# NVIDIA/nvidia-resiliency-ext

Measured on AMD Instinct MI355X. Metric: generate_report_latency_us, lower is better.
Workload: dtype f32; 1 GPU; 8 ranks x 64 sections x 10000 samples per report, ring capacity 10000, relative+individual scores, gather_on_rank0; logical_ranks_per_gpu=8, rows_per_gpu=512, exchange=none (single process)

## Files before the change

### include/nvrx_straggler.h

```cpp
#ifndef NVRX_STRAGGLER_H
#define NVRX_STRAGGLER_H

#include <stddef.h>
#include <stdint.h>

#ifdef __cplusplus
extern "C" {
#endif

#define NVRX_ABI_VERSION 2

#define NVRX_OK 0
#define NVRX_ERR_INVALID (-22)
#define NVRX_ERR_NOMEM (-12)
#define NVRX_ERR_HIP (-5)
#define NVRX_ERR_STATE (-1)
#define NVRX_ERR_RANGE (-34)
#define NVRX_ERR_TIMEOUT (-62)

#define NVRX_STATS_STRIDE 8
#define NVRX_STAT_MIN 0
#define NVRX_STAT_MAX 1
#define NVRX_STAT_MED 2
#define NVRX_STAT_AVG 3
// ... 175 lines not shown
    float *d_stats_dst;
    uint32_t *d_done_counter;
    void *allgather_fn;
    void *comm;
    int32_t send_count;
    uint32_t seq;
    const uint32_t *h_seq_word;
    double timeout_s;
    void *order_after_stream;
    int32_t order_after_enabled;
    int32_t resident;
    int32_t prev_settled;
    int32_t guard_rings;
} nvrx_report_desc;
int nvrx_report(nvrx_ctx *ctx, nvrx_report_desc *desc, void *stream);
int nvrx_report_attribute(nvrx_ctx *ctx, const nvrx_report_desc *desc, int first_rank, int n_ranks, int top_n, void *d_out);
int nvrx_tail_local(nvrx_ctx *ctx, const nvrx_report_desc *desc, uint32_t q_ppm, float *d_tail_send, int K, int S,
                    int rows_active, void *stream);
int nvrx_onset_enable(nvrx_ctx *ctx, int on);
int nvrx_onset_local(nvrx_ctx *ctx, const nvrx_report_desc *desc, uint32_t min_seg_ppm, float min_strength,
                     float *d_onset_send, int K, int S, int rows_active, void *stream);
int nvrx_period_local(nvrx_ctx *ctx, const nvrx_report_desc *desc, int max_period, float min_strength,
                      float *d_period_send, int K, int S, int rows_active, void *stream);
int nvrx_episode_local(nvrx_ctx *ctx, const nvrx_report_desc *desc, uint32_t min_len_ppm, float min_strength,
                       float *d_episode_send, int K, int S, int rows_active, void *stream);
int nvrx_report_robust(nvrx_ctx *ctx, const nvrx_report_desc *desc, int first_rank, int n_ranks, int min_ranks,
                       float floor_rel, void *d_out);
int nvrx_report_peer(nvrx_ctx *ctx, const nvrx_report_desc *desc, const int32_t *d_groups, int G, int first_rank, int n_ranks,
                     int min_ranks, void *d_out);
int nvrx_report_pace(nvrx_ctx *ctx, const nvrx_report_desc *desc, int first_rank, int n_ranks, int min_ranks, void *d_out);
// ... 15 lines not shown
#define NVRX_WINDOW_MISS 1
#define NVRX_WINDOW_NAMES 2
typedef struct nvrx_window_desc {
    int (*kt_sync)(double timeout_s);
    int (*kt_hold)(int on);
    uint64_t (*kt_counter)(int what);
    double kt_patience_s;
    uint64_t kt_rows_known;
    uint64_t kt_keys_without_row;
    int32_t rows_used;
    int32_t asynchronous;
    int32_t harvest_regions;
    int32_t out_names_ok;
} nvrx_window_desc;
int nvrx_window_report(nvrx_ctx *ctx, nvrx_report_desc *desc, void *stream, nvrx_window_desc *window);
int nvrx_window_clocks(double *out2);
int nvrx_report_clocks(double *out8);
int nvrx_report_desc_size(void);
typedef struct nvrx_peer nvrx_peer;
int nvrx_peer_create(int device, int world, int rank, int max_floats_per_rank, nvrx_peer **out);
int nvrx_peer_ipc_handle(nvrx_peer *peer, void *handle64 );
int nvrx_peer_connect(nvrx_peer *peer, int peer_rank, const void *handle64);
int nvrx_peer_device_id(const nvrx_peer *peer, char *out, int len);
int nvrx_peer_check_access(const nvrx_peer *peer, int peer_rank, const char *peer_pci_bus_id);
int nvrx_peer_ready(nvrx_peer *peer, double timeout_s);
int nvrx_peer_allgather(const void *send, void *recv, size_t count, int dtype, void *comm, void *stream);
void *nvrx_peer_allgather_address(void);
int nvrx_peer_error(const nvrx_peer *peer, uint32_t *epoch_out);
int nvrx_peer_destroy(nvrx_peer *peer);

// ... 19 lines not shown
```

### nvidia-resiliency-ext_amd/csrc/nvrx_straggler.hip

```cpp
#include <hip/hip_runtime.h>
#include <hip/hip_ext.h>

#include <algorithm>
#include <atomic>
#include <chrono>
#include <thread>
#include <cmath>
#include <cstdarg>
#include <cstdio>
#include <cstdlib>
#include <cstring>
#include <deque>
#include <mutex>
#include <string>
#include <unordered_map>
#include <utility>
#include <vector>

#include "nvrx_straggler.h"

namespace {

thread_local std::string g_err;

// ... 1691 lines not shown
    hipEvent_t order_ev = nullptr;
    hipStream_t score_stream = nullptr;
    unsigned long long *d_rowg = nullptr;
    uint32_t *h_gather_err = nullptr, *d_gather_err = nullptr;
    uint32_t gran_epoch = 0;
    int wall_khz = 100000;
    int resident_mode = 1;
    int poll_naps = 4;
    int rehome_mode = 1;
    bool side_work = true;
    uint64_t reports_rehomed = 0;
    int last_rehome_verdict = 0;
    uint64_t side_gen = 1, async_gen = 0;
    bool async_on_ctx = false;
    double last_report_us = 0.0;
    double async_rehome_gap_us = 5000.0;
    hipEvent_t report_ev = nullptr;
    uint64_t report_epoch = 0;
    hipStream_t guard_stream = nullptr;
    bool guard_recorded = true;
    bool stamps_used = false;
    uint64_t guard_done_epoch = 0;
    struct StreamEpoch {
        hipStream_t stream;
        uint64_t epoch;
    };
    std::vector<StreamEpoch> stream_epochs;

    const nvrx_report_desc *attr_desc = nullptr;
    hipStream_t attr_stream = nullptr;
// ... 1171 lines not shown
    a->rank = p->rank;
    a->count = (int)count;
    a->stride = p->stride;
    p->epoch = (p->epoch % 0x7FFFFFFFu) + 1u;
    a->epoch = p->epoch;
    a->timeout_ticks = (unsigned long long)(p->timeout_s * 1e3 * (double)p->wall_khz);
    return NVRX_OK;
}

int nvrx_report_clocks(double *out8) {
    if (!out8) return fail(NVRX_ERR_INVALID, "null argument");
    memcpy(out8, g_report_clk, sizeof(g_report_clk));
    return NVRX_OK;
}

int nvrx_report(nvrx_ctx *ctx, nvrx_report_desc *d, void *stream) {
    report_clk(0);
    if (!ctx || !d) return fail(NVRX_ERR_INVALID, "null argument");
    if (!d->d_stats || !d->d_send || !d->d_scores || !d->d_meta) return fail(NVRX_ERR_INVALID, "null buffer in the report descriptor");
    const bool exchanging = d->allgather_fn != nullptr;
    if (exchanging && (!d->d_table || d->d_table == d->d_send || d->send_count <= 0))
        return fail(NVRX_ERR_INVALID, "an exchange needs a separate table buffer and a positive send_count");
    const bool is_async = d->h_seq_word == nullptr;
    bool async_gap_ok = false;
    {
        std::lock_guard<std::mutex> lk(ctx->mu);
        const double now_us = g_report_clk[0];
        async_gap_ok = ctx->async_rehome_gap_us > 0.0 && ctx->last_report_us > 0.0 && now_us - ctx->last_report_us >= ctx->async_rehome_gap_us;
        ctx->last_report_us = now_us;
        ctx->last_rehome_verdict = 0;
        if (d->prev_settled) {
            ctx->guard_done_epoch = ctx->report_epoch;
            if (ctx->async_on_ctx && ctx->async_gen == ctx->side_gen) ctx->side_work = false;
            ctx->async_on_ctx = false;
        }
    }
    bool rehomed = false;
    if (ctx->rehome_mode && ((!is_async && !d->guard_rings) || (is_async && d->guard_rings && async_gap_ok))) {
        std::lock_guard<std::mutex> lk(ctx->mu);
        hipStream_t only = nullptr;
        int distinct = 0;
// ... 88 lines not shown
        ga.timeout_ticks = (unsigned long long)((d->timeout_s > 0.0 ? d->timeout_s : 1e9) * 1e3 * (double)ctx->wall_khz);
        ga.poll_naps = ctx->poll_naps;
        PeerArgs pa{};
        if (peer_route) {
            rc2 = peer_fill_args(static_cast<nvrx_peer *>(d->comm), d->d_send, d->d_table, (size_t)d->send_count, &pa);
            if (rc2) return rc2;
        }
        d->seq = (d->seq % 0x7FFFFFFFu) + 1u;
        rc2 = score_launch(exchanging ? d->d_table : d->d_send, d->R, d->K, d->S, d->do_indiv, d->do_rel, d->thresholds,
                           d->d_scores, d->d_flags, d->d_meta, d->d_done_counter, d->seq, nullptr, nullptr, 0,
                           ctx->score_stream, peer_route ? &pa : nullptr, &ga);
        if (rc2) return rc2;
        ctx->attr_desc = d, ctx->attr_stream = ctx->score_stream;
        report_clk(4);
        report_clk(5);
        rc2 = nvrx_poll_u32(d->h_seq_word, d->seq, d->timeout_s > 0.0 ? d->timeout_s : 1e30);
        report_clk(6);
        if (rc2) return rc2;
        if (*static_cast<volatile uint32_t *>(ctx->h_gather_err) == ctx->gran_epoch)
            return fail(NVRX_ERR_TIMEOUT, "the score kernel gave up waiting for the statistics kernel's rows (epoch %u)", ctx->gran_epoch);
        if (as_stream(stream) == ctx->default_stream) {
            std::lock_guard<std::mutex> lk(ctx->mu);
            ctx->side_work = false;
            ctx->async_on_ctx = false;
        }
        return NVRX_OK;
    }
    int rc = report_local_impl(ctx, d->d_stats, d->d_send, d->K, d->S, d->names_ok, d->rows_active, stream, nullptr, 0);
    if (rc) return rc;
    if (d->guard_rings) {
        std::lock_guard<std::mutex> lk(ctx->mu);
        ctx->guard_stream = as_stream(stream);
        if (rehomed || !ctx->stamps_used) {
            ctx->guard_recorded = false;
        } else {
            HIP_TRY(hipEventRecord(ctx->report_ev, as_stream(stream)));
            ctx->guard_recorded = true;
        }
        ctx->report_epoch++;
    }
// ... 9 lines not shown
        const int nrc = reinterpret_cast<AllGatherFn>(d->allgather_fn)(d->d_send, d->d_table, (size_t)d->send_count, 7,
                                                                       d->comm, stream);
        if (nrc != 0) {
            return fail(NVRX_ERR_HIP, "all-gather of the exchange rows failed (ncclResult %d)", nrc);
        }
    }
    report_clk(4);
    d->seq = (d->seq % 0x7FFFFFFFu) + 1u;
    rc = score_launch(exchanging ? d->d_table : d->d_send, d->R, d->K, d->S, d->do_indiv, d->do_rel, d->thresholds,
                      d->d_scores, d->d_flags, d->d_meta, d->d_done_counter, d->seq, d->d_stats, d->d_stats_dst,
                      d->stats_rows, stream, prologue ? &pa : nullptr);
    if (rc) return rc;
    ctx->attr_desc = d, ctx->attr_stream = as_stream(stream);
    report_clk(5);
    if (d->h_seq_word) {
        rc = nvrx_poll_u32(d->h_seq_word, d->seq, d->timeout_s > 0.0 ? d->timeout_s : 1e30);
        report_clk(6);
        if (rc == NVRX_OK && !rehomed && as_stream(stream) == ctx->default_stream) {
            std::lock_guard<std::mutex> lk(ctx->mu);
            ctx->side_work = false;
            ctx->async_on_ctx = false;
        }
        return rc;
    }
    if (!rehomed) {
        std::lock_guard<std::mutex> lk(ctx->mu);
        ctx->async_on_ctx = true;
        ctx->async_gen = ctx->side_gen;
    }
    return NVRX_OK;
}

static thread_local double g_window_clk[2] = {0.0, 0.0};

int nvrx_window_clocks(double *out2) {
    if (!out2) return fail(NVRX_ERR_INVALID, "out2 is null");
    out2[0] = g_window_clk[0], out2[1] = g_window_clk[1];
    return NVRX_OK;
}

int nvrx_window_report(nvrx_ctx *ctx, nvrx_report_desc *desc, void *stream, nvrx_window_desc *w) {
    if (!ctx || !desc || !w) return fail(NVRX_ERR_INVALID, "null argument");
    g_window_clk[0] = g_window_clk[1] = std::chrono::duration<double, std::micro>(std::chrono::steady_clock::now().time_since_epoch()).count();
    const bool per_kernel = w->kt_sync != nullptr;
    if (per_kernel && (!w->kt_hold || !w->kt_counter)) return fail(NVRX_ERR_INVALID, "a kernel tracer needs sync, hold and counter");
    const bool enqueue_only = w->asynchronous != 0;
    bool held = false;
    auto leave = [&](int rc) {
        if (held) w->kt_hold(0);
        return rc;
    };
    w->out_names_ok = 1;
    if (per_kernel) {
        if (enqueue_only) {
            w->kt_hold(1);
            held = true;
// ... 11 lines not shown
    {
        const int n = w->rows_used;
        bool bad = false, changed = false;
        {
            std::lock_guard<std::mutex> lk(ctx->mu);
            bad = n < 0 || n > ctx->rows;
            if (!bad) {
                changed = ctx->occupied_rows != n;
                for (int r = 0; r < n && !changed; r++) changed = ctx->occupied_seen[(size_t)r] != (uint8_t)(ctx->total[(size_t)r] != 0);
            }
        }
        if (bad) return leave(fail(NVRX_ERR_INVALID, "rows_used %d outside [0,%d]", n, ctx->rows));
        if (changed) return leave(NVRX_WINDOW_MISS);
    }
    g_window_clk[1] = std::chrono::duration<double, std::micro>(std::chrono::steady_clock::now().time_since_epoch()).count();
    const int rc = nvrx_report(ctx, desc, stream);
    if (rc < 0) return leave(rc);
    if (!enqueue_only && desc->h_seq_word) {
        const uint32_t names = *const_cast<const volatile uint32_t *>(desc->h_seq_word - 4);
        if (names != 1u) {
            w->out_names_ok = 0;
            return leave(NVRX_WINDOW_NAMES);
        }
    }
    const int rrc = nvrx_ring_reset(ctx);
    return leave(rrc < 0 ? rrc : NVRX_OK);
}

int nvrx_peer_create(int device, int world, int rank, int max_floats_per_rank, nvrx_peer **out) {
    if (!out) return fail(NVRX_ERR_INVALID, "out is null");
// ... 275 lines not shown
```

### nvidia-resiliency-ext_amd/nvrx_straggler/_native.py

```python
from __future__ import annotations

import ctypes
import os
import threading
from ctypes import POINTER, c_char_p, c_double, c_float, c_int, c_int32, c_size_t, c_uint32, c_uint64, c_void_p

_LIB_NAME = "libnvrx_straggler_hip.so"
_LIB_PATH = os.path.join(os.environ.get("NVRX_DEBUG_LIB_DIR") or os.path.join(os.path.dirname(os.path.abspath(__file__)), "lib"), _LIB_NAME)

NVRX_ABI_VERSION = 2
STATS_STRIDE = 8
STAT_MIN, STAT_MAX, STAT_MED, STAT_AVG, STAT_STD, STAT_NUM, STAT_WEIGHT = range(7)
KIND_SECTION, KIND_KERNEL = 0, 1
MAX_RING_CAP = 65536
META_WORDS = 8
ERR_TIMEOUT = -62
ERR_RANGE = -34
ERR_INVALID = -22
ERR_STATE = -1
ATTR_MAX_TOP = 16
TAIL_Q_PPM_MIN, TAIL_Q_PPM_MAX = 500000, 999999
ROUTE_SINGLE, ROUTE_ROWS, ROUTE_ROWS_PRE, ROUTE_TILE16, ROUTE_TILE8 = 1, 2, 3, 4, 5
ROBUST_MAX_RANKS = 65536
PEER_MAX_GROUPS = 4096
# ... 89 lines not shown
    ("nvrx_row_configure", c_int, [c_void_p, c_int, c_int, c_int]),
    ("nvrx_ring_push", c_int, [c_void_p, c_int, c_float]),
    ("nvrx_ring_push_many", c_int, [c_void_p, c_int, c_void_p, c_int]),
    ("nvrx_ring_push_pairs", c_int, [c_void_p, c_void_p, c_void_p, c_int]),
    ("nvrx_ring_push_staged", c_int, [c_void_p, c_void_p, c_void_p, c_int]),
    ("nvrx_sink_push", c_int, [c_void_p, c_void_p, c_void_p, c_int]),
    ("nvrx_sink_row_alloc", c_int, [c_void_p, c_int]),
    ("nvrx_ring_push_device", c_int, [c_void_p, c_int, c_void_p, c_int, c_void_p]),
    ("nvrx_ring_push_device_rows", c_int, [c_void_p, c_int, c_int, c_void_p, c_int, c_int, c_void_p]),
    ("nvrx_ring_set_count", c_int, [c_void_p, c_int, c_int]),
    ("nvrx_ring_set_count_all", c_int, [c_void_p, c_int]),
    ("nvrx_ring_count", c_int, [c_void_p, c_int]),
    ("nvrx_ring_counts", c_int, [c_void_p, c_void_p, c_int]),
    ("nvrx_ring_occupancy_changed", c_int, [c_void_p, c_int]),
    ("nvrx_window_report", c_int, [c_void_p, c_void_p, c_void_p, c_void_p]),
    ("nvrx_window_clocks", c_int, [POINTER(c_double)]),
    ("nvrx_ring_reset", c_int, [c_void_p]),
    ("nvrx_history_reset", c_int, [c_void_p, c_void_p]),
    ("nvrx_ring_flush", c_int, [c_void_p, c_void_p]),
    ("nvrx_ring_read", c_int, [c_void_p, c_int, c_void_p, c_int, c_void_p]),
    ("nvrx_event_begin", c_int, [c_void_p, c_int, c_void_p]),
    ("nvrx_event_end", c_int, [c_void_p, c_int, c_void_p]),
    ("nvrx_event_harvest", c_int, [c_void_p, c_int]),
    ("nvrx_stamp_begin", c_int, [c_void_p, c_int, c_void_p]),
    ("nvrx_stamp_end", c_int, [c_void_p, c_int, c_int, c_float, c_void_p]),
    ("nvrx_report_local", c_int, [c_void_p, c_void_p, c_void_p, c_int, c_int, c_int, c_int, c_void_p]),
    ("nvrx_report", c_int, [c_void_p, POINTER(ReportDesc), c_void_p]),
    ("nvrx_report_attribute", c_int, [c_void_p, POINTER(ReportDesc), c_int, c_int, c_int, c_void_p]),
    ("nvrx_tail_local", c_int, [c_void_p, POINTER(ReportDesc), c_uint32, c_void_p, c_int, c_int, c_int, c_void_p]),
    ("nvrx_onset_enable", c_int, [c_void_p, c_int]),
    ("nvrx_onset_local", c_int, [c_void_p, POINTER(ReportDesc), c_uint32, c_float, c_void_p, c_int, c_int, c_int, c_void_p]),
    ("nvrx_period_local", c_int, [c_void_p, POINTER(ReportDesc), c_int, c_float, c_void_p, c_int, c_int, c_int, c_void_p]),
    ("nvrx_episode_local", c_int, [c_void_p, POINTER(ReportDesc), c_uint32, c_float, c_void_p, c_int, c_int, c_int, c_void_p]),
    ("nvrx_report_robust", c_int, [c_void_p, POINTER(ReportDesc), c_int, c_int, c_int, c_float, c_void_p]),
    ("nvrx_report_peer", c_int, [c_void_p, POINTER(ReportDesc), c_void_p, c_int, c_int, c_int, c_int, c_void_p]),
    ("nvrx_report_pace", c_int, [c_void_p, POINTER(ReportDesc), c_int, c_int, c_int, c_void_p]),
    ("nvrx_report_pace_group", c_int, [c_void_p, POINTER(ReportDesc), c_void_p, c_int, c_int, c_int, c_int, c_int, c_int,
                                       c_void_p]),
    ("nvrx_report_node", c_int, [c_void_p, POINTER(ReportDesc), c_void_p, c_int, c_int, c_int, c_int, c_int, c_int, c_void_p]),
    ("nvrx_report_history", c_int, [c_void_p, POINTER(ReportDesc), c_int, c_int, c_void_p, c_int, c_int, c_uint64,
                                    POINTER(c_double), c_void_p]),
    ("nvrx_report_trend", c_int, [c_void_p, c_void_p, c_int, c_int, c_int, c_int, c_uint64, c_void_p]),
# ... 225 lines not shown
```

### nvidia-resiliency-ext_amd/nvrx_straggler/backend.py

```python
from __future__ import annotations

import ctypes
import os
import threading
import weakref
from typing import Any, Dict, List, Optional, Sequence

import numpy as np
import torch

from . import _native
from .row_families import EPISODE, FAMILIES, ONSET, PERIOD, TAIL, RowFamily
from .table_families import NODE, PACE, PACE_GROUP, PEER, ROBUST, SLOTS, TableFamily

DEFAULT_THRESHOLDS = (0.75, 0.75, 0.75, 0.75)



def report_timeout_s() -> float:
    t = _timeout_cache[0]
    if t is None:
        t = refresh_report_timeout()
    return t

# ... 1399 lines not shown
        d.rows_active, d.stats_rows = rows_active, min(stats_rows, ws.stats_rows)
        d.do_indiv, d.do_rel = int(do_indiv), int(do_rel)
        d.names_ok = int(names_ok)
        for i in range(4):
            d.thresholds[i] = float(thresholds[i])
        if direct is not None:
            d.allgather_fn, d.comm = direct.fn_address, direct.comm_address
        else:
            d.allgather_fn, d.comm = None, None
        d.timeout_s = report_timeout_s()
        d.h_seq_word = blk.h_seq if wait else None
        d.guard_rings = 0 if wait else 1
        d.resident = 1 if (wait and resident) else 0
        blk.desc_key = key

    def report_fused(self, ws: Workspace, rows_active: int, stats_rows: int, do_indiv: bool, do_rel: bool,
                     thresholds: Sequence[float], direct=None, names_ok: bool = True, wait: bool = True,
                     order_after: Optional[int] = None, resident: bool = True, prev_settled: bool = False) -> int:
        blk = ws.flip()
        d = blk.desc
        key = (rows_active, stats_rows, do_indiv, do_rel, thresholds, direct, names_ok, wait, resident)
        if blk.desc_key != key:
            self.configure_desc(ws, blk, key)
        d.prev_settled = 1 if (prev_settled and not wait) else 0
        if order_after is not None:
            d.order_after_stream, d.order_after_enabled = order_after, 1
        elif d.order_after_enabled:
            d.order_after_enabled = 0
        if not ws.send_initialised:
            self.backend.send_init(ws)
            self.backend.synchronize()
        d.seq = ws.seq
        rc = self.lib.nvrx_report(self.ctx, blk.desc_ref, self.backend._stream_handle)
        ws.seq = d.seq
        if rc < 0:
            if rc == _native.ERR_TIMEOUT:
                self.backend.retire_workspace(ws)
            _native.check(rc)
        return ws.seq

    def report_attribute(self, ws: Workspace, top_n: int, first_rank: int = 0, n_ranks: Optional[int] = None) -> Attribution:
        n_ranks = ws.R - first_rank if n_ranks is None else n_ranks
        ws.attr_settle()
        buf, _ = ws.attr_buffers(n_ranks, top_n, False)
        rc = self.lib.nvrx_report_attribute(self.ctx, ws.block.desc_ref, first_rank, n_ranks, top_n, buf.data_ptr())
        if rc < 0:
            _native.check(rc)
        out = ws._attr_last = Attribution(self.backend, buf, first_rank, n_ranks, top_n)
        return out

    def _table_report(self, fam: TableFamily, ws: Workspace, groups: Optional[PeerGroups], first_rank: int,
                      n_ranks: Optional[int], params: tuple) -> TableScores:
        return self.backend._table_step(fam, ws, getattr(self.lib, fam.c_report), (self.ctx, ws.block.desc_ref), (), groups,
                                        first_rank, n_ranks, params)
# ... 127 lines not shown
```

### nvidia-resiliency-ext_amd/nvrx_straggler/reporting.py

```python
from __future__ import annotations

import collections
import dataclasses
import itertools
import logging
import math
import os
import threading
import time
from typing import Any, Dict, List, Mapping, Optional, Sequence

import numpy as np

from . import backend as _backend_mod
from . import dist_utils, row_families
from .name_mapper import NameMapper, name_digest
from .statistics import NUM_COLUMN, STAT_KEYS, Statistic

_SummaryType = Mapping[Statistic, float]
_LOG = logging.getLogger(__name__)



def _load_pyread():
# ... 1597 lines not shown
        self.rank = dist_utils.get_rank(self.group)
        self.node_name = node_name
        self.thresholds = tuple(float(t) for t in thresholds)

        self.min_local_kernel_times: Dict[str, float] = collections.defaultdict(lambda: float("inf"))
        self.min_local_section_times: Dict[str, float] = collections.defaultdict(lambda: float("inf"))

        self.name_mapper = NameMapper(pg=pg)
        self._private_mapper = NameMapper(pg=pg)
        self.rank_to_node: Dict[int, str] = collections.defaultdict(lambda: "<unk>")
        self._rank_to_node_folded = False
        self._direct = None
        self._direct_tried = False
        self.asynchronous = bool(asynchronous)
        self.exchange_info: Dict[str, Any] = {}
        self._ring_plan = None
        self._ring_gid_state = None
        self._inflight: Optional[_PendingBlock] = None
        self._prev_async_settled = True
        self._resync_pending = False
        self._had_ring_report = False
        self._unreported_rows: list = []
        n = int(kernel_attribution)
        if not 0 <= n <= 16:
            raise ValueError(f"kernel_attribution must be 0 (off) or 1..16 kernels per GPU score, got {kernel_attribution!r}")
        self.kernel_attribution = n
        if n:
            be = _backend_mod._backend
            if be is not None and not hasattr(be, "attribute"):
                raise RuntimeError(f"kernel_attribution={n}: the active backend ({getattr(be, 'name', type(be).__name__)}) "
# ... 658 lines not shown
            raise RuntimeError("peer_groups: these rings run the one-call report but have no report_peer")
        if fused and self.pace_scores and not hasattr(rings, "report_pace_group" if self.pace_peer_groups else "report_pace"):
            if self.pace_peer_groups:
                raise RuntimeError("pace_peer_groups: these rings run the one-call report but have no report_pace_group")
            raise RuntimeError("pace_scores: these rings run the one-call report but have no report_pace")
        if fused and self.node_scores and not hasattr(rings, "report_node"):
            raise RuntimeError("node_scores: these rings run the one-call report but have no report_node")
        if fused and self._peer_history is not None and not hasattr(rings, "report_peer_history"):
            raise RuntimeError("peer_history: these rings run the one-call report but have no report_peer_history")
        if fused and self.peer_trends and not hasattr(rings, "report_peer_trend"):
            raise RuntimeError("peer_trends: these rings run the one-call report but have no report_peer_trend")
        if fused and self._history is not None and not hasattr(rings, "report_history"):
            raise RuntimeError("score_history: these rings run the one-call report but have no report_history")
        if fused and self.score_trends and not hasattr(rings, "report_trend"):
            raise RuntimeError("score_trends: these rings run the one-call report but have no report_trend")
        if fused:
            wait = not self.asynchronous
            seq = rings.report_fused(ws, plan.rows_used, plan.stats_needed, self.is_computing_indiv_scores,
                                     self.is_computing_rel_scores, self.thresholds, self._direct if multi else None,
                                     names_ok=names_ok, wait=wait, order_after=order_after if multi else None,
                                     resident=not (multi and getattr(self._direct, "shared_device", False)
                                                   and os.environ.get("NVRX_DEBUG_RESIDENT_SHARED_OK", "0") in ("", "0")),
                                     prev_settled=self._prev_async_settled)
            if not wait:
                self._prev_async_settled = False
                pend = self._inflight = _PendingBlock(be, ws, seq)
                if self.gather_on_rank0 and self.rank != 0:
                    return None
                report = Report._from_device(
                    _ScoreSource(plan.view, pend),
                    self._shared_rank_to_node(),
                    (time.perf_counter_ns() - t0) * 1e-6, self.gather_on_rank0, self.rank)
                if attr_n:
                    self._attach_plan_attribution(report, plan, rings, True)
                if self.robust_scores:
                    self._attach_plan_robust(report, plan, rings, True)
                if self.work_groups:
                    self._attach_plan_work(report, plan, rings, True)
                if self.peer_groups is not None:
                    self._attach_plan_peer(report, plan, rings, True)
                if self.pace_scores:
                    self._attach_plan_pace(report, plan, rings, True)
                if self.node_scores:
                    self._attach_plan_node(report, plan, rings, True)
                if self._history is not None:
                    self._attach_plan_history(report, plan, rings, True)
                return report
        else:
            rings.report_local(ws, True, rows_active=plan.rows_used)
            table = self._exchange(be, ws) if multi else ws.send
            be.score(ws, table, self.is_computing_indiv_scores, self.is_computing_rel_scores, self.thresholds,
                     wait=True, stats_rows=plan.stats_needed)
        if fused:
            mark = getattr(ws, "mark_live", None)
            if mark is not None:
                mark(ws.seq)
        if multi:
            self._check_exchange()
        if ws.meta[0] != 1:
            return False
        if self.gather_on_rank0 and self.rank != 0:
            return None
        if fused:
            pending = _LiveBlock(be, ws, ws.seq, plan.stats_needed)
            ws.attach(pending)
        else:
            pending = ws.host_block()
        report = Report._from_device(
            _ScoreSource(plan.view, pending),
            self._shared_rank_to_node(),
            (time.perf_counter_ns() - t0) * 1e-6, self.gather_on_rank0, self.rank)
        if attr_n:
            self._attach_plan_attribution(report, plan, rings, fused)
        if self.robust_scores:
            self._attach_plan_robust(report, plan, rings, fused)
        if self.work_groups:
            self._attach_plan_work(report, plan, rings, fused)
        if self.peer_groups is not None:
            self._attach_plan_peer(report, plan, rings, fused)
        if self.pace_scores:
            self._attach_plan_pace(report, plan, rings, fused)
        if self.node_scores:
            self._attach_plan_node(report, plan, rings, fused)
        if self._history is not None:
            self._attach_plan_history(report, plan, rings, fused)
        return report
# ... 368 lines not shown
```

### nvidia-resiliency-ext_amd/nvrx_straggler/straggler.py

```python
from __future__ import annotations

import ctypes
import dataclasses
import functools
import inspect
import logging
import os
import socket
import sys
import time
from collections.abc import Callable
from contextlib import contextmanager
from typing import Any, Dict, Iterable, List, Optional, Sequence, Union

from . import _native, row_families
from . import backend as _backend_mod
from . import dist_utils as _dist_utils
from . import ktrace as _ktrace
from .cupti import CuptiManager
from .interval_tracker import ReportIntervalTracker
from .reporting import Report, ReportGenerator, _LiveBlock, _PendingBlock, _ScoreSource
from .statistics import Statistic

GPU_KEY_PREFIX = "hipevent::"
# ... 57 lines not shown
        self.row = rings.row_for(_native.KIND_SECTION, name)
        self.gpu_row: Optional[int] = None
        self.cpu_elapsed_times = _ElapsedRing(rings, self.row)


_MISS = object()
_TRACED_DISPATCH_US = 1.0


class _Lane:

    trace = None

    __slots__ = ("rings", "reporter", "manager", "ext", "plan", "ws", "be", "view", "versions", "wr", "group", "wr_cache",
                 "rows_used", "desc_key", "window", "window_ref", "call", "ctx", "stream", "multi", "enqueue_only",
                 "returns_none", "stats_needed", "gather_on_rank0", "rank", "token", "asynchronous")

    @classmethod
    def build(cls, det) -> Optional["_Lane"]:
        rings, reporter, manager = det._rings, det.reporter, det._cupti_manager
        plan = reporter._ring_plan
        call = getattr(getattr(rings, "lib", None), "nvrx_window_report", None)
        if plan is None or not plan.fused or call is None or manager is None or not manager.is_initialized:
            return None
        multi = reporter.world_size > 1 and reporter._exchanged()
        if (multi and reporter._direct is None) or det._pending_region_switch is not None:
            return None
        if reporter.asynchronous and not reporter.enqueue_only():
            return None
        if reporter.kernel_attribution:
            return None
# ... 37 lines not shown
        if manager.per_kernel:
            if not getattr(ext, "_counting", False):
                return None
            cast, klib = ctypes.cast, ext._lib
            w.kt_sync = cast(klib.nvrx_ktrace_sync, ctypes.c_void_p).value
            w.kt_hold = cast(klib.nvrx_ktrace_hold, ctypes.c_void_p).value
            w.kt_counter = cast(klib.nvrx_ktrace_counter, ctypes.c_void_p).value
            w.kt_patience_s = float(ext.sync_patience_s)
            w.kt_rows_known, w.kt_keys_without_row = int(ext._rows_known), int(ext.keys_without_row)
        else:
            w.harvest_regions = 1
        w.rows_used = self.rows_used
        w.asynchronous = 1 if self.enqueue_only else 0
        self.window_ref = ctypes.byref(w)
        self.call, self.ctx, self.stream = call, rings.ctx, self.be._stream_handle
        return self

    def run(self, det):
        t0 = time.perf_counter_ns()
        tr = _Lane.trace
        reporter, ws, rings = self.reporter, self.ws, self.rings
        if (reporter._ring_plan is not self.plan or rings._rows_used != self.rows_used or reporter._resync_pending
                or reporter.asynchronous is not self.asynchronous
                or (reporter.name_mapper.version, reporter._private_mapper.version) != self.versions
                or _dist_utils.world_and_rank(self.group, self.wr_cache) != self.wr):
            return _MISS
        if self.enqueue_only:
            pend = reporter._inflight
            if pend is not None:
                blk = pend.blk
# ... 16 lines not shown
        if nxt.desc_key != self.desc_key:
            rings.configure_desc(ws, nxt, self.desc_key)
        if nxt._live is not None:
            nxt.settle()
        ws._cur, ws.block = 1 - cur, nxt
        d = nxt.desc
        if self.enqueue_only:
            d.prev_settled = 1 if reporter._prev_async_settled else 0
        if self.multi:
            d.order_after_stream, d.order_after_enabled = self.be.current_stream_handle(), 1
        elif d.order_after_enabled:
            d.order_after_enabled = 0
        d.seq = ws.seq
        if tr is not None:
            tr.append(("settle_flip_desc", time.perf_counter_ns() - t0))
        rc = self.call(self.ctx, nxt.desc_ref, self.stream, self.window_ref)
        if tr is not None:
            tr.append(("c_call", time.perf_counter_ns() - t0))
        seq = ws.seq = d.seq
        if rc == _native.WINDOW_MISS:
            ws._cur, ws.block = cur, ws.blocks[cur]
            return _MISS
        if rc < 0:
            reporter._drop_plan()
            if rc == _native.ERR_TIMEOUT:
                self.be.retire_workspace(ws)
            _native.check(rc)
        if self.enqueue_only:
            reporter._prev_async_settled = False
            pend = reporter._inflight = _PendingBlock(self.be, ws, seq)
# ... 5 lines not shown
        if self.multi:
            reporter._check_exchange()
        if rc == _native.WINDOW_NAMES:
            reporter._sync_names_first()
            return det._report_and_reset(rings, reporter)
        if self.returns_none:
            return None
        live = _LiveBlock(self.be, ws, seq, self.stats_needed)
        nxt.attach(live)
        if tr is not None:
            tr.append(("live_block", time.perf_counter_ns() - t0))
        rep = Report._from_device(_ScoreSource(self.view, live), reporter._shared_rank_to_node(),
                                  (time.perf_counter_ns() - t0) * 1e-6, self.gather_on_rank0, self.rank)
        if tr is not None:
            tr.append(("report_object", time.perf_counter_ns() - t0))
        return rep


def _peer_groups_from_env(value: str, name: str = "NVRX_PEER_GROUPS"):
    value = value.strip()
    if not value:
        return None
    if ":" in value or value == "auto":
        return value
    try:
        return [int(x) for x in value.split(",")]
    except ValueError:
        raise ValueError(f"{name} must be 'block:N', 'mod:N' or a comma-separated list of integers, "
                         f"got {value!r}") from None

# ... 629 lines not shown
```

Measured before the change: 26.24 us.

## Split synchronous report into enqueue and wait to overlap host object construction

Splits nvrx_report and nvrx_window_report into enqueue and wait/finish halves, keeping per-context pending state. The Python lane and reporter now enqueue the GPU report, build the Report and live-block objects while the kernels run, and only then poll the completion word. This hides the host-side Python object construction behind GPU execution. The cost is extra state-machine complexity, a new error path when a wait is missed, and the need for try/finally cleanup.

```diff
diff --git a/include/nvrx_straggler.h b/include/nvrx_straggler.h
--- a/include/nvrx_straggler.h
+++ b/include/nvrx_straggler.h
@@ -213,6 +213,8 @@
     int32_t guard_rings;
 } nvrx_report_desc;
 int nvrx_report(nvrx_ctx *ctx, nvrx_report_desc *desc, void *stream);
+int nvrx_report_enqueue(nvrx_ctx *ctx, nvrx_report_desc *desc, void *stream);
+int nvrx_report_wait(nvrx_ctx *ctx, nvrx_report_desc *desc);
 int nvrx_report_attribute(nvrx_ctx *ctx, const nvrx_report_desc *desc, int first_rank, int n_ranks, int top_n, void *d_out);
 int nvrx_tail_local(nvrx_ctx *ctx, const nvrx_report_desc *desc, uint32_t q_ppm, float *d_tail_send, int K, int S,
                     int rows_active, void *stream);
@@ -258,6 +260,8 @@
     int32_t out_names_ok;
 } nvrx_window_desc;
 int nvrx_window_report(nvrx_ctx *ctx, nvrx_report_desc *desc, void *stream, nvrx_window_desc *window);
+int nvrx_window_enqueue(nvrx_ctx *ctx, nvrx_report_desc *desc, void *stream, nvrx_window_desc *window);
+int nvrx_window_finish(nvrx_ctx *ctx, nvrx_report_desc *desc, nvrx_window_desc *window);
 int nvrx_window_clocks(double *out2);
 int nvrx_report_clocks(double *out8);
 int nvrx_report_desc_size(void);
diff --git a/nvidia-resiliency-ext_amd/csrc/nvrx_straggler.hip b/nvidia-resiliency-ext_amd/csrc/nvrx_straggler.hip
--- a/nvidia-resiliency-ext_amd/csrc/nvrx_straggler.hip
+++ b/nvidia-resiliency-ext_amd/csrc/nvrx_straggler.hip
@@ -1729,6 +1729,10 @@
     uint64_t side_gen = 1, async_gen = 0;
     bool async_on_ctx = false;
     double last_report_us = 0.0;
+    bool pend_on = false;
+    bool pend_resident = false, pend_rehomed = false;
+    hipStream_t pend_stream = nullptr;
+    uint32_t pend_seq = 0;
     double async_rehome_gap_us = 5000.0;
     hipEvent_t report_ev = nullptr;
     uint64_t report_epoch = 0;
@@ -2930,7 +2934,54 @@
     return NVRX_OK;
 }
 
+static void report_set_pending(nvrx_ctx *ctx, const nvrx_report_desc *d, bool resident, bool rehomed, hipStream_t st) {
+    std::lock_guard<std::mutex> lk(ctx->mu);
+    ctx->pend_on = true;
+    ctx->pend_resident = resident, ctx->pend_rehomed = rehomed;
+    ctx->pend_stream = st;
+    ctx->pend_seq = d->seq;
+}
+
 int nvrx_report(nvrx_ctx *ctx, nvrx_report_desc *d, void *stream) {
+    const int rc = nvrx_report_enqueue(ctx, d, stream);
+    if (rc || !d->h_seq_word) return rc;
+    return nvrx_report_wait(ctx, d);
+}
+
+int nvrx_report_wait(nvrx_ctx *ctx, nvrx_report_desc *d) {
+    if (!ctx || !d) return fail(NVRX_ERR_INVALID, "null argument");
+    if (!d->h_seq_word) return NVRX_OK;
+    bool resident = false, rehomed = false;
+    hipStream_t st = nullptr;
+    uint32_t seq = 0;
+    {
+        std::lock_guard<std::mutex> lk(ctx->mu);
+        if (!ctx->pend_on) return fail(NVRX_ERR_STATE, "nvrx_report_wait: no enqueued report is waiting on this context");
+        resident = ctx->pend_resident, rehomed = ctx->pend_rehomed, st = ctx->pend_stream, seq = ctx->pend_seq;
+        ctx->pend_on = false;
+    }
+    int rc = nvrx_poll_u32(d->h_seq_word, seq, d->timeout_s > 0.0 ? d->timeout_s : 1e30);
+    report_clk(6);
+    if (resident) {
+        if (rc) return rc;
+        if (*static_cast<volatile uint32_t *>(ctx->h_gather_err) == ctx->gran_epoch)
+            return fail(NVRX_ERR_TIMEOUT, "the score kernel gave up waiting for the statistics kernel's rows (epoch %u)", ctx->gran_epoch);
+        if (st == ctx->default_stream) {
+            std::lock_guard<std::mutex> lk(ctx->mu);
+            ctx->side_work = false;
+            ctx->async_on_ctx = false;
+        }
+        return NVRX_OK;
+    }
+    if (rc == NVRX_OK && !rehomed && st == ctx->default_stream) {
+        std::lock_guard<std::mutex> lk(ctx->mu);
+        ctx->side_work = false;
+        ctx->async_on_ctx = false;
+    }
+    return rc;
+}
+
+int nvrx_report_enqueue(nvrx_ctx *ctx, nvrx_report_desc *d, void *stream) {
     report_clk(0);
     if (!ctx || !d) return fail(NVRX_ERR_INVALID, "null argument");
     if (!d->d_stats || !d->d_send || !d->d_scores || !d->d_meta) return fail(NVRX_ERR_INVALID, "null buffer in the report descriptor");
@@ -2941,6 +2992,8 @@
     bool async_gap_ok = false;
     {
         std::lock_guard<std::mutex> lk(ctx->mu);
+        if (ctx->pend_on)
+            return fail(NVRX_ERR_STATE, "report %u was enqueued on this context and has not been waited for (nvrx_report_wait)", ctx->pend_seq);
         const double now_us = g_report_clk[0];
         async_gap_ok = ctx->async_rehome_gap_us > 0.0 && ctx->last_report_us > 0.0 && now_us - ctx->last_report_us >= ctx->async_rehome_gap_us;
         ctx->last_report_us = now_us;
@@ -3059,16 +3112,7 @@
         ctx->attr_desc = d, ctx->attr_stream = ctx->score_stream;
         report_clk(4);
         report_clk(5);
-        rc2 = nvrx_poll_u32(d->h_seq_word, d->seq, d->timeout_s > 0.0 ? d->timeout_s : 1e30);
-        report_clk(6);
-        if (rc2) return rc2;
-        if (*static_cast<volatile uint32_t *>(ctx->h_gather_err) == ctx->gran_epoch)
-            return fail(NVRX_ERR_TIMEOUT, "the score kernel gave up waiting for the statistics kernel's rows (epoch %u)", ctx->gran_epoch);
-        if (as_stream(stream) == ctx->default_stream) {
-            std::lock_guard<std::mutex> lk(ctx->mu);
-            ctx->side_work = false;
-            ctx->async_on_ctx = false;
-        }
+        report_set_pending(ctx, d, true, rehomed, as_stream(stream));
         return NVRX_OK;
     }
     int rc = report_local_impl(ctx, d->d_stats, d->d_send, d->K, d->S, d->names_ok, d->rows_active, stream, nullptr, 0);
@@ -3108,14 +3152,8 @@
     ctx->attr_desc = d, ctx->attr_stream = as_stream(stream);
     report_clk(5);
     if (d->h_seq_word) {
-        rc = nvrx_poll_u32(d->h_seq_word, d->seq, d->timeout_s > 0.0 ? d->timeout_s : 1e30);
-        report_clk(6);
-        if (rc == NVRX_OK && !rehomed && as_stream(stream) == ctx->default_stream) {
-            std::lock_guard<std::mutex> lk(ctx->mu);
-            ctx->side_work = false;
-            ctx->async_on_ctx = false;
-        }
-        return rc;
+        report_set_pending(ctx, d, false, rehomed, as_stream(stream));
+        return NVRX_OK;
     }
     if (!rehomed) {
         std::lock_guard<std::mutex> lk(ctx->mu);
@@ -3133,7 +3171,35 @@
     return NVRX_OK;
 }
 
+static int window_report_impl(nvrx_ctx *ctx, nvrx_report_desc *desc, void *stream, nvrx_window_desc *w, bool finish);
+
 int nvrx_window_report(nvrx_ctx *ctx, nvrx_report_desc *desc, void *stream, nvrx_window_desc *w) {
+    return window_report_impl(ctx, desc, stream, w, true);
+}
+
+int nvrx_window_enqueue(nvrx_ctx *ctx, nvrx_report_desc *desc, void *stream, nvrx_window_desc *w) {
+    if (!ctx || !desc || !w) return fail(NVRX_ERR_INVALID, "null argument");
+    if (w->asynchronous != 0 || !desc->h_seq_word)
+        return fail(NVRX_ERR_INVALID, "nvrx_window_enqueue is for synchronous windows (asynchronous ones: nvrx_window_report)");
+    return window_report_impl(ctx, desc, stream, w, false);
+}
+
+int nvrx_window_finish(nvrx_ctx *ctx, nvrx_report_desc *desc, nvrx_window_desc *w) {
+    if (!ctx || !desc || !w) return fail(NVRX_ERR_INVALID, "null argument");
+    if (w->asynchronous != 0 || !desc->h_seq_word)
+        return fail(NVRX_ERR_INVALID, "nvrx_window_finish is for synchronous windows (asynchronous ones: nvrx_window_report)");
+    const int rc = nvrx_report_wait(ctx, desc);
+    if (rc < 0) return rc;
+    const uint32_t names = *const_cast<const volatile uint32_t *>(desc->h_seq_word - 4);
+    if (names != 1u) {
+        w->out_names_ok = 0;
+        return NVRX_WINDOW_NAMES;
+    }
+    const int rrc = nvrx_ring_reset(ctx);
+    return rrc < 0 ? rrc : NVRX_OK;
+}
+
+static int window_report_impl(nvrx_ctx *ctx, nvrx_report_desc *desc, void *stream, nvrx_window_desc *w, bool finish) {
     if (!ctx || !desc || !w) return fail(NVRX_ERR_INVALID, "null argument");
     g_window_clk[0] = g_window_clk[1] = std::chrono::duration<double, std::micro>(std::chrono::steady_clock::now().time_since_epoch()).count();
     const bool per_kernel = w->kt_sync != nullptr;
@@ -3175,6 +3241,7 @@
         if (changed) return leave(NVRX_WINDOW_MISS);
     }
     g_window_clk[1] = std::chrono::duration<double, std::micro>(std::chrono::steady_clock::now().time_since_epoch()).count();
+    if (!finish) return leave(nvrx_report_enqueue(ctx, desc, stream));
     const int rc = nvrx_report(ctx, desc, stream);
     if (rc < 0) return leave(rc);
     if (!enqueue_only && desc->h_seq_word) {
diff --git a/nvidia-resiliency-ext_amd/csrc/split_report_args_check.cpp b/nvidia-resiliency-ext_amd/csrc/split_report_args_check.cpp
--- /dev/null
+++ b/nvidia-resiliency-ext_amd/csrc/split_report_args_check.cpp
@@ -0,0 +1,60 @@
+#include "args_check.h"
+
+static int sync_stub(double) { return 0; }
+
+int main() {
+    nvrx_ctx *ctx = reinterpret_cast<nvrx_ctx *>(uintptr_t{4096});
+    float *buf = reinterpret_cast<float *>(uintptr_t{8192});
+    uint32_t word[8] = {0, 0, 0, 0, 0, 0, 0, 0};
+    nvrx_report_desc d;
+    memset(&d, 0, sizeof(d));
+    nvrx_window_desc w;
+    memset(&w, 0, sizeof(w));
+
+    expect("enqueue null ctx", nvrx_report_enqueue(nullptr, &d, nullptr), NVRX_ERR_INVALID, "null");
+    expect("enqueue null desc", nvrx_report_enqueue(ctx, nullptr, nullptr), NVRX_ERR_INVALID, "null");
+    expect("enqueue null buffers", nvrx_report_enqueue(ctx, &d, nullptr), NVRX_ERR_INVALID, "null buffer");
+    expect("report null buffers", nvrx_report(ctx, &d, nullptr), NVRX_ERR_INVALID, "null buffer");
+    d.d_stats = d.d_send = d.d_scores = buf;
+    expect("enqueue null meta", nvrx_report_enqueue(ctx, &d, nullptr), NVRX_ERR_INVALID, "null buffer");
+    d.d_meta = reinterpret_cast<uint32_t *>(buf);
+    d.allgather_fn = reinterpret_cast<void *>(&sync_stub);
+    expect("enqueue exchange without a table", nvrx_report_enqueue(ctx, &d, nullptr), NVRX_ERR_INVALID, "table");
+    d.d_table = d.d_send;
+    d.send_count = 8;
+    expect("enqueue exchange into the send rows", nvrx_report_enqueue(ctx, &d, nullptr), NVRX_ERR_INVALID, "table");
+    d.d_table = buf + 1024;
+    d.send_count = 0;
+    expect("enqueue exchange of nothing", nvrx_report_enqueue(ctx, &d, nullptr), NVRX_ERR_INVALID, "send_count");
+    d.allgather_fn = nullptr;
+
+    expect("wait null ctx", nvrx_report_wait(nullptr, &d), NVRX_ERR_INVALID, "null");
+    expect("wait null desc", nvrx_report_wait(ctx, nullptr), NVRX_ERR_INVALID, "null");
+    d.h_seq_word = nullptr;
+    expect("wait on an asynchronous descriptor", nvrx_report_wait(ctx, &d), NVRX_OK, nullptr);
+
+    d.h_seq_word = &word[4];
+    expect("window enqueue null ctx", nvrx_window_enqueue(nullptr, &d, nullptr, &w), NVRX_ERR_INVALID, "null");
+    expect("window enqueue null desc", nvrx_window_enqueue(ctx, nullptr, nullptr, &w), NVRX_ERR_INVALID, "null");
+    expect("window enqueue null window", nvrx_window_enqueue(ctx, &d, nullptr, nullptr), NVRX_ERR_INVALID, "null");
+    w.asynchronous = 1;
+    expect("window enqueue asynchronous", nvrx_window_enqueue(ctx, &d, nullptr, &w), NVRX_ERR_INVALID, "synchronous");
+    w.asynchronous = 0;
+    d.h_seq_word = nullptr;
+    expect("window enqueue without a completion word", nvrx_window_enqueue(ctx, &d, nullptr, &w), NVRX_ERR_INVALID, "synchronous");
+    d.h_seq_word = &word[4];
+    w.kt_sync = &sync_stub;
+    expect("window enqueue half a tracer", nvrx_window_enqueue(ctx, &d, nullptr, &w), NVRX_ERR_INVALID, "tracer");
+    w.kt_sync = nullptr;
+
+    expect("window finish null ctx", nvrx_window_finish(nullptr, &d, &w), NVRX_ERR_INVALID, "null");
+    expect("window finish null desc", nvrx_window_finish(ctx, nullptr, &w), NVRX_ERR_INVALID, "null");
+    expect("window finish null window", nvrx_window_finish(ctx, &d, nullptr), NVRX_ERR_INVALID, "null");
+    w.asynchronous = 1;
+    expect("window finish asynchronous", nvrx_window_finish(ctx, &d, &w), NVRX_ERR_INVALID, "synchronous");
+    w.asynchronous = 0;
+    d.h_seq_word = nullptr;
+    expect("window finish without a completion word", nvrx_window_finish(ctx, &d, &w), NVRX_ERR_INVALID, "synchronous");
+    printf("split_report_args_check: %d failure(s)\n", failures);
+    return failures ? 1 : 0;
+}
diff --git a/nvidia-resiliency-ext_amd/nvrx_straggler/_native.py b/nvidia-resiliency-ext_amd/nvrx_straggler/_native.py
--- a/nvidia-resiliency-ext_amd/nvrx_straggler/_native.py
+++ b/nvidia-resiliency-ext_amd/nvrx_straggler/_native.py
@@ -127,6 +127,8 @@
     ("nvrx_ring_counts", c_int, [c_void_p, c_void_p, c_int]),
     ("nvrx_ring_occupancy_changed", c_int, [c_void_p, c_int]),
     ("nvrx_window_report", c_int, [c_void_p, c_void_p, c_void_p, c_void_p]),
+    ("nvrx_window_enqueue", c_int, [c_void_p, c_void_p, c_void_p, c_void_p]),
+    ("nvrx_window_finish", c_int, [c_void_p, c_void_p, c_void_p]),
     ("nvrx_window_clocks", c_int, [POINTER(c_double)]),
     ("nvrx_ring_reset", c_int, [c_void_p]),
     ("nvrx_history_reset", c_int, [c_void_p, c_void_p]),
@@ -139,6 +141,8 @@
     ("nvrx_stamp_end", c_int, [c_void_p, c_int, c_int, c_float, c_void_p]),
     ("nvrx_report_local", c_int, [c_void_p, c_void_p, c_void_p, c_int, c_int, c_int, c_int, c_void_p]),
     ("nvrx_report", c_int, [c_void_p, POINTER(ReportDesc), c_void_p]),
+    ("nvrx_report_enqueue", c_int, [c_void_p, POINTER(ReportDesc), c_void_p]),
+    ("nvrx_report_wait", c_int, [c_void_p, POINTER(ReportDesc)]),
     ("nvrx_report_attribute", c_int, [c_void_p, POINTER(ReportDesc), c_int, c_int, c_int, c_void_p]),
     ("nvrx_tail_local", c_int, [c_void_p, POINTER(ReportDesc), c_uint32, c_void_p, c_int, c_int, c_int, c_void_p]),
     ("nvrx_onset_enable", c_int, [c_void_p, c_int]),
diff --git a/nvidia-resiliency-ext_amd/nvrx_straggler/backend.py b/nvidia-resiliency-ext_amd/nvrx_straggler/backend.py
--- a/nvidia-resiliency-ext_amd/nvrx_straggler/backend.py
+++ b/nvidia-resiliency-ext_amd/nvrx_straggler/backend.py
@@ -1437,12 +1437,9 @@
         d.resident = 1 if (wait and resident) else 0
         blk.desc_key = key
 
-    def report_fused(self, ws: Workspace, rows_active: int, stats_rows: int, do_indiv: bool, do_rel: bool,
-                     thresholds: Sequence[float], direct=None, names_ok: bool = True, wait: bool = True,
-                     order_after: Optional[int] = None, resident: bool = True, prev_settled: bool = False) -> int:
+    def _report_arm(self, ws: Workspace, key: tuple, wait: bool, order_after: Optional[int], prev_settled: bool) -> ResultBlock:
         blk = ws.flip()
         d = blk.desc
-        key = (rows_active, stats_rows, do_indiv, do_rel, thresholds, direct, names_ok, wait, resident)
         if blk.desc_key != key:
             self.configure_desc(ws, blk, key)
         d.prev_settled = 1 if (prev_settled and not wait) else 0
@@ -1454,13 +1451,40 @@
             self.backend.send_init(ws)
             self.backend.synchronize()
         d.seq = ws.seq
+        return blk
+
+    def report_fused(self, ws: Workspace, rows_active: int, stats_rows: int, do_indiv: bool, do_rel: bool,
+                     thresholds: Sequence[float], direct=None, names_ok: bool = True, wait: bool = True,
+                     order_after: Optional[int] = None, resident: bool = True, prev_settled: bool = False) -> int:
+        blk = self._report_arm(ws, (rows_active, stats_rows, do_indiv, do_rel, thresholds, direct, names_ok, wait, resident),
+                               wait, order_after, prev_settled)
         rc = self.lib.nvrx_report(self.ctx, blk.desc_ref, self.backend._stream_handle)
-        ws.seq = d.seq
+        ws.seq = blk.desc.seq
         if rc < 0:
             if rc == _native.ERR_TIMEOUT:
                 self.backend.retire_workspace(ws)
             _native.check(rc)
         return ws.seq
+
+    def report_enqueue(self, ws: Workspace, rows_active: int, stats_rows: int, do_indiv: bool, do_rel: bool,
+                       thresholds: Sequence[float], direct=None, names_ok: bool = True, order_after: Optional[int] = None,
+                       resident: bool = True) -> int:
+        blk = self._report_arm(ws, (rows_active, stats_rows, do_indiv, do_rel, thresholds, direct, names_ok, True, resident),
+                               True, order_after, False)
+        rc = self.lib.nvrx_report_enqueue(self.ctx, blk.desc_ref, self.backend._stream_handle)
+        ws.seq = blk.desc.seq
+        if rc < 0:
+            if rc == _native.ERR_TIMEOUT:
+                self.backend.retire_workspace(ws)
+            _native.check(rc)
+        return ws.seq
+
+    def report_wait(self, ws: Workspace) -> None:
+        rc = self.lib.nvrx_report_wait(self.ctx, ws.block.desc_ref)
+        if rc < 0:
+            if rc == _native.ERR_TIMEOUT:
+                self.backend.retire_workspace(ws)
+            _native.check(rc)
 
     def report_attribute(self, ws: Workspace, top_n: int, first_rank: int = 0, n_ranks: Optional[int] = None) -> Attribution:
         n_ranks = ws.R - first_rank if n_ranks is None else n_ranks
diff --git a/nvidia-resiliency-ext_amd/nvrx_straggler/reporting.py b/nvidia-resiliency-ext_amd/nvrx_straggler/reporting.py
--- a/nvidia-resiliency-ext_amd/nvrx_straggler/reporting.py
+++ b/nvidia-resiliency-ext_amd/nvrx_straggler/reporting.py
@@ -1635,6 +1635,7 @@
         self._direct_tried = False
         self.asynchronous = bool(asynchronous)
         self.exchange_info: Dict[str, Any] = {}
+        self._split_report = os.environ.get("NVRX_DEBUG_SPLIT_REPORT", "1") not in ("0",)
         self._ring_plan = None
         self._ring_gid_state = None
         self._inflight: Optional[_PendingBlock] = None
@@ -2323,14 +2324,32 @@
             raise RuntimeError("score_history: these rings run the one-call report but have no report_history")
         if fused and self.score_trends and not hasattr(rings, "report_trend"):
             raise RuntimeError("score_trends: these rings run the one-call report but have no report_trend")
-        if fused:
+        report = None
+        resident = fused and not (multi and getattr(self._direct, "shared_device", False)
+                                  and os.environ.get("NVRX_DEBUG_RESIDENT_SHARED_OK", "0") in ("", "0"))
+        if (fused and self._split_report and not self.asynchronous and not (self.gather_on_rank0 and self.rank != 0)
+                and hasattr(rings, "report_enqueue")):
+            rings.report_enqueue(ws, plan.rows_used, plan.stats_needed, self.is_computing_indiv_scores,
+                                 self.is_computing_rel_scores, self.thresholds, self._direct if multi else None,
+                                 names_ok=names_ok, order_after=order_after if multi else None, resident=resident)
+            attached = False
+            try:
+                pending = _LiveBlock(be, ws, ws.seq, plan.stats_needed)
+                ws.attach(pending)
+                attached = True
+                report = Report._from_device(_ScoreSource(plan.view, pending), self._shared_rank_to_node(), 0.0,
+                                             self.gather_on_rank0, self.rank)
+            finally:
+                rings.report_wait(ws)
+                if not attached:
+                    ws.mark_live(ws.seq)
+            report.__dict__["generate_report_elapsed_time"] = (time.perf_counter_ns() - t0) * 1e-6
+        elif fused:
             wait = not self.asynchronous
             seq = rings.report_fused(ws, plan.rows_used, plan.stats_needed, self.is_computing_indiv_scores,
                                      self.is_computing_rel_scores, self.thresholds, self._direct if multi else None,
                                      names_ok=names_ok, wait=wait, order_after=order_after if multi else None,
-                                     resident=not (multi and getattr(self._direct, "shared_device", False)
-                                                   and os.environ.get("NVRX_DEBUG_RESIDENT_SHARED_OK", "0") in ("", "0")),
-                                     prev_settled=self._prev_async_settled)
+                                     resident=resident, prev_settled=self._prev_async_settled)
             if not wait:
                 self._prev_async_settled = False
                 pend = self._inflight = _PendingBlock(be, ws, seq)
@@ -2360,7 +2379,7 @@
             table = self._exchange(be, ws) if multi else ws.send
             be.score(ws, table, self.is_computing_indiv_scores, self.is_computing_rel_scores, self.thresholds,
                      wait=True, stats_rows=plan.stats_needed)
-        if fused:
+        if fused and report is None:
             mark = getattr(ws, "mark_live", None)
             if mark is not None:
                 mark(ws.seq)
@@ -2370,15 +2389,16 @@
             return False
         if self.gather_on_rank0 and self.rank != 0:
             return None
-        if fused:
-            pending = _LiveBlock(be, ws, ws.seq, plan.stats_needed)
-            ws.attach(pending)
-        else:
-            pending = ws.host_block()
-        report = Report._from_device(
-            _ScoreSource(plan.view, pending),
-            self._shared_rank_to_node(),
-            (time.perf_counter_ns() - t0) * 1e-6, self.gather_on_rank0, self.rank)
+        if report is None:
+            if fused:
+                pending = _LiveBlock(be, ws, ws.seq, plan.stats_needed)
+                ws.attach(pending)
+            else:
+                pending = ws.host_block()
+            report = Report._from_device(
+                _ScoreSource(plan.view, pending),
+                self._shared_rank_to_node(),
+                (time.perf_counter_ns() - t0) * 1e-6, self.gather_on_rank0, self.rank)
         if attr_n:
             self._attach_plan_attribution(report, plan, rings, fused)
         if self.robust_scores:
diff --git a/nvidia-resiliency-ext_amd/nvrx_straggler/straggler.py b/nvidia-resiliency-ext_amd/nvrx_straggler/straggler.py
--- a/nvidia-resiliency-ext_amd/nvrx_straggler/straggler.py
+++ b/nvidia-resiliency-ext_amd/nvrx_straggler/straggler.py
@@ -95,7 +95,7 @@
 
     __slots__ = ("rings", "reporter", "manager", "ext", "plan", "ws", "be", "view", "versions", "wr", "group", "wr_cache",
                  "rows_used", "desc_key", "window", "window_ref", "call", "ctx", "stream", "multi", "enqueue_only",
-                 "returns_none", "stats_needed", "gather_on_rank0", "rank", "token", "asynchronous")
+                 "returns_none", "stats_needed", "gather_on_rank0", "rank", "token", "asynchronous", "enqueue", "finish")
 
     @classmethod
     def build(cls, det) -> Optional["_Lane"]:
@@ -163,6 +163,10 @@
         w.asynchronous = 1 if self.enqueue_only else 0
         self.window_ref = ctypes.byref(w)
         self.call, self.ctx, self.stream = call, rings.ctx, self.be._stream_handle
+        self.enqueue = self.finish = None
+        if getattr(reporter, "_split_report", False) and not self.enqueue_only and not self.returns_none:
+            self.enqueue = getattr(rings.lib, "nvrx_window_enqueue", None)
+            self.finish = getattr(rings.lib, "nvrx_window_finish", None)
         return self
 
     def run(self, det):
@@ -209,6 +213,8 @@
         d.seq = ws.seq
         if tr is not None:
             tr.append(("settle_flip_desc", time.perf_counter_ns() - t0))
+        if self.enqueue is not None:
+            return self._run_split(det, t0, tr, cur, nxt)
         rc = self.call(self.ctx, nxt.desc_ref, self.stream, self.window_ref)
         if tr is not None:
             tr.append(("c_call", time.perf_counter_ns() - t0))
@@ -244,6 +250,49 @@
                                   (time.perf_counter_ns() - t0) * 1e-6, self.gather_on_rank0, self.rank)
         if tr is not None:
             tr.append(("report_object", time.perf_counter_ns() - t0))
+        return rep
+
+    def _run_split(self, det, t0, tr, cur, nxt):
+        reporter, ws, rings = self.reporter, self.ws, self.rings
+        rc = self.enqueue(self.ctx, nxt.desc_ref, self.stream, self.window_ref)
+        if tr is not None:
+            tr.append(("enqueue", time.perf_counter_ns() - t0))
+        seq = ws.seq = nxt.desc.seq
+        if rc == _native.WINDOW_MISS:
+            ws._cur, ws.block = cur, ws.blocks[cur]
+            return _MISS
+        if rc < 0:
+            reporter._drop_plan()
+            if rc == _native.ERR_TIMEOUT:
+                self.be.retire_workspace(ws)
+            _native.check(rc)
+        rep = None
+        try:
+            live = _LiveBlock(self.be, ws, seq, self.stats_needed)
+            nxt.attach(live)
+            rep = Report._from_device(_ScoreSource(self.view, live), reporter._shared_rank_to_node(), 0.0, self.gather_on_rank0,
+                                      self.rank)
+            del live
+            if tr is not None:
+                tr.append(("objects_built", time.perf_counter_ns() - t0))
+        finally:
+            rc = self.finish(self.ctx, nxt.desc_ref, self.window_ref)
+            if tr is not None:
+                tr.append(("word_seen", time.perf_counter_ns() - t0))
+            if rep is None:
+                nxt.mark_live(seq)
+            if rc < 0:
+                reporter._drop_plan()
+                if rc == _native.ERR_TIMEOUT:
+                    self.be.retire_workspace(ws)
+                _native.check(rc)
+        if self.multi:
+            reporter._check_exchange()
+        if rc == _native.WINDOW_NAMES:
+            del rep
+            reporter._sync_names_first()
+            return det._report_and_reset(rings, reporter)
+        rep.__dict__["generate_report_elapsed_time"] = (time.perf_counter_ns() - t0) * 1e-6
         return rep
 
 
```

Measured after the change: 25.26 us (median of 5 runs). 3.7% less time.
